# Damo12320/OptixPathtracer

Hardware: AMD Instinct MI355X
Metric: Msamples/sec at 1920x1080, max-depth 8; MSE vs reference (higher is better)
Workload: dtype f32; 1 GPU; BASELINE configs[1]: Diffuse sphere-in-box 1920x1080, 1024 spp, depth 8, 1xMI355X; scene=sphere_box_diffuse, triangles=34570, width=1920, height=1080, max_depth=8, material_mode=lambert, kernel=auto (wavefront), frames_per_launch=128, wavefront_streams=1, parallelism=spp-shard x1, batch_frames=128, queue_bytes=55207544320, queue_budget_bytes=77305217024, bvh_builder=auto (GPU binned SAH + GPU SAH-optimal BVH4 collapse), primary_dedup=True

## Files before the change

optixpathtracer_amd/csrc/pt_device.h:

```cpp
#pragma once
#include "pt_bsdf.h"

namespace pt {

constexpr int kEmptyChild = (int)0x80000000;

struct __align__(16) BNode4 {
    float4 lox, hix, loy, hiy, loz, hiz;
    int4 child;
    int4 pad;
};

__device__ __forceinline__ int leaf_first(int c) { return (~c) >> 3; }
__device__ __forceinline__ int leaf_count(int c) { return ((~c) & 7) + 1; }

struct DevScene {
    const BNode4* nodes;
    const float4* isect;
    const float4* shade;
    const float4* mats;
    const float4* tuv;
    const uint32_t* texels;
    const int4* texinfo;
    int ntri;
// ... 531 lines not shown
                s.h.back = code < 0;
                s.h.orig = ow;
            }
            L->key[lane] = ~0ull;
        }
        __builtin_amdgcn_wave_barrier();
    }
}

template <int ANY, bool STATS, int DEPTH>
__device__ __forceinline__ bool trav_node_step(const DevScene& S, TravState& s, int* __restrict__ stk, int stride,
                                               int* spill, TravStats& ts) {
    if (s.cur >= 0) {
        if (STATS) {
            ts.nodes++;
            ts.lds_nodes += s.cur < S.n_lds;
        }
        float t0, t1, t2, t3;
        int c0, c1, c2, c3;
        const NodeLoad nl = node_load(S, s, s.cur);
#if PT_CYCLE_PROBE
        if (STATS) ts.probe_t = probe_clock(nl.ch.x);
#endif
        node_eval(nl, s, t0, t1, t2, t3, c0, c1, c2, c3);
        if (ANY != kRayAny) {
            cswap(t0, c0, t1, c1);
            cswap(t2, c2, t3, c3);
            cswap(t0, c0, t2, c2);
            cswap(t1, c1, t3, c3);
            cswap(t1, c1, t2, c2);
        }
        if (s.sp > DEPTH - 3) stack_spill<DEPTH, STATS>(s, stk, stride, spill, ts);
        {
            int sp = s.sp;
            stk[sp * stride] = c3;
            sp += c3 != kEmptyChild;
            stk[sp * stride] = c2;
            sp += c2 != kEmptyChild;
            stk[sp * stride] = c1;
            sp += c1 != kEmptyChild;
            s.sp = sp;
        }
        s.cur = c0;
    }
    if (s.cur == kEmptyChild) stack_pop<DEPTH>(s, stk, stride, spill);
    if (s.cur < 0 && s.cur != kEmptyChild && s.leaf == kEmptyChild) {
        s.leaf = s.cur;
        stack_pop<DEPTH>(s, stk, stride, spill);
    }
    return s.cur == kEmptyChild && s.leaf == kEmptyChild;
}

template <int ANY>
__device__ __forceinline__ bool trav_hit_acceptable(const TravState& s, const float4 A, const float4 E1,
                                                    const float4 E2) {
    const float t = is_any<ANY>(s) ? __int_as_float(s.path) : s.h.t;
    return tri_accept(A, E1, E2, s.inv, s.io, t);
}
template <int ANY, bool TEX>
__device__ __forceinline__ bool trav_result_ok(const DevScene& S, const TravState& s) {
    if (s.strict || s.h.tri < 0) return true;
    const int ti = s.h.tri;
    return trav_hit_acceptable<ANY>(s, S.isect[3 * ti], S.isect[3 * ti + 1], S.isect[3 * ti + 2]);
}

template <int ANY>
__device__ __forceinline__ void trav_restart_strict(TravState& s, float tmax_closest) {
    s.cur = 0;
    s.sp = 0;
    s.spc = 0;
    s.leaf = kEmptyChild;
    s.strict = true;
    s.h.tri = -1;
    if (!is_any<ANY>(s)) {
        s.best = tmax_closest;
        s.h.orig = 0x7fffffff;
    }
}

template <int ANY, bool STATS, int DEPTH, bool TEX>
__device__ __forceinline__ bool traverse(const DevScene& S, f3 o, f3 d, float tmin, float tmax, Hit& h,
                                         int* __restrict__ stk, int stride, TravStats& ts) {
    if (STATS) ts.rays++;
    TravState s;
    trav_init(s, o, d, tmin, tmax);
    if (S.ntri > 0) {
        int spill[kSpillDepth];
        while (true) {
            while (!trav_step<ANY, STATS, DEPTH, TEX>(S, s, stk, stride, spill, ts)) {
            }
            if (trav_result_ok<ANY, TEX>(S, s)) break;
            if (STATS) ts.retrace++;
            trav_restart_strict<ANY>(s, tmax);
        }
    }
    h = s.h;
    return s.h.tri >= 0;
}

__device__ __forceinline__ void camera_ray(const DevLaunch& L, int x, int y, f3& o, f3& d) {
    float xs = ((float)x + 0.5f) / (float)L.width;
    float ys = ((float)(y + L.row0) + 0.5f) / (float)L.image_height;
    float ndc[4] = {xs * 2.0f - 1.0f, ys * 2.0f - 1.0f, 1.0f, 1.0f};
    float pv[4], pw[4];
    mat4_mul_vec4(L.inv_proj, ndc, pv);
    float pv0[4] = {pv[0], pv[1], pv[2], 0.0f};
    mat4_mul_vec4(L.inv_view, pv0, pw);
    float d4 = (pw[0] * pw[0] + pw[1] * pw[1]) + (pw[2] * pw[2] + pw[3] * pw[3]);
    float inv = 1.0f / sqrtf(d4);
    d = mk(pw[0] * inv, pw[1] * inv, pw[2] * inv);
    o = mk(L.cam_pos[0], L.cam_pos[1], L.cam_pos[2]);
}

struct SurfaceHit {
    f3 pos, ng;
    Frame fr;
    f3 wo;
    f3 albedo;
    float metallic, roughness;
};

__device__ __forceinline__ void apply_textures(const DevScene& S, int ti, float u, float v, const float4 M1,
                                               const float4 M2, f3& albedo, float& metallic, float& roughness,
                                               f3& Ns) {
    const int at = __float_as_int(M1.z), nt = __float_as_int(M1.w), mt = __float_as_int(M2.x);
    float x, y;
    tri_texcoord(S, ti, u, v, x, y);
    f3 ntex = mk(0.0f, 0.0f, 0.0f);
    if (at >= 0) {
        const float4 c = tex_sample(S, at, x, y, true);
        albedo = albedo * mk(c.x, c.y, c.z);
    }
    if (nt >= 0) {
        const float4 c = tex_sample(S, nt, x, y, false);
        ntex = mk(c.x, c.y, c.z);
    }
    if (mt >= 0) {
        const float4 c = tex_sample(S, mt, x, y, false);
        metallic = c.x;
        roughness = c.y;
    }
    if (ntex.x != 0.0f || ntex.y != 0.0f || ntex.z != 0.0f) {
        f3 d1 = cross(Ns, mk(0.0f, 0.0f, 1.0f));
        f3 d2 = cross(Ns, mk(0.0f, 1.0f, 0.0f));
        f3 T0 = (length(d1) > length(d2)) ? d1 : d2;
        T0 = normalize(T0);
        const f3 B0 = cross(T0, Ns);
        const f3 tn = mk(ntex.x * 2.0f - 1.0f, ntex.y * 2.0f - 1.0f, ntex.z * 2.0f - 1.0f);
        Ns = normalize(mk((T0.x * tn.x + B0.x * tn.y) + Ns.x * tn.z, (T0.y * tn.x + B0.y * tn.y) + Ns.y * tn.z,
                          (T0.z * tn.x + B0.z * tn.y) + Ns.z * tn.z));
    }
}

template <bool TEX>
__device__ __forceinline__ void reconstruct(const DevScene& S, const Hit& h, f3 d, SurfaceHit& s) {
    const int ti = h.tri;
    const float4 A = S.isect[3 * ti];
    const float4 S0 = S.shade[4 * ti], S1 = S.shade[4 * ti + 1], S2 = S.shade[4 * ti + 2], S3 = S.shade[4 * ti + 3];
    const float4 E1 = make_float4(S0.x - A.x, S0.y - A.y, S0.z - A.z, 0.0f);
    const float4 E2 = make_float4(S1.x - A.x, S1.y - A.y, S1.z - A.z, 0.0f);
    const int mi = __float_as_int(S3.w);
    const float4 M0 = S.mats[kMatStride * mi], M1 = S.mats[kMatStride * mi + 1];
    f3 wo_w = normalize(-d);
    f3 v0 = mk(A.x, A.y, A.z), v1 = mk(S0.x, S0.y, S0.z), v2 = mk(S1.x, S1.y, S1.z);
    f3 n0 = mk(S0.w, S1.w, S2.x), n1 = mk(S2.y, S2.z, S2.w), n2 = mk(S3.x, S3.y, S3.z);
    f3 Ng = cross(mk(E1.x, E1.y, E1.z), mk(E2.x, E2.y, E2.z));
    const float u = h.u, v = h.v;
    float w = 1.0f - u - v;
    f3 Ns = mk(w * n0.x + u * n1.x + v * n2.x, w * n0.y + u * n1.y + v * n2.y, w * n0.z + u * n1.z + v * n2.z);
    if (M1.y != kNormalNone) {
        if (TEX && M1.y == kNormalObject) {
            const float4 R0 = S.mats[kMatStride * mi + 3], R1 = S.mats[kMatStride * mi + 4],
                         R2 = S.mats[kMatStride * mi + 5];
            Ns = mk(mat_row_dir(R0, Ns), mat_row_dir(R1, Ns), mat_row_dir(R2, Ns));
        }
        Ns = normalize(Ns);
    }
    if (dot(wo_w, Ng) < 0.0f) Ng = -Ng;
    Ng = normalize(Ng);
    if (dot(Ng, Ns) < 0.0f) Ns = -Ns;
    Ns = normalize(Ns);
    if (h.back) {
        Ns = Ns * -1.0f;
        Ng = Ng * -1.0f;
    }
    s.pos = mk(w * v0.x + u * v1.x + v * v2.x, w * v0.y + u * v1.y + v * v2.y, w * v0.z + u * v1.z + v * v2.z);
    s.ng = Ng;
    s.albedo = mk(M0.x, M0.y, M0.z);
    s.metallic = M0.w;
    s.roughness = M1.x;
    if (TEX) {
        const float4 M2 = S.mats[kMatStride * mi + 2];
        if (M2.y != 0.0f) apply_textures(S, ti, u, v, M1, M2, s.albedo, s.metallic, s.roughness, Ns);
    }
    f3 c1 = cross(Ns, mk(0.0f, 0.0f, 1.0f));
    f3 c2 = cross(Ns, mk(0.0f, 1.0f, 0.0f));
    f3 T = (length(c1) > length(c2)) ? c1 : c2;
    T = normalize(T);
    s.fr.t = T;
    s.fr.b = cross(T, Ns);
    s.fr.n = Ns;
    s.wo = to_local(s.fr, wo_w);
}

struct PathState {
    f3 o, d, beta, radiance;
    uint32_t seed;
    int bounce;
    bool end;
};

__device__ __forceinline__ void path_start(PathState& p, f3 o, f3 d, uint32_t seed) {
    p.o = o;
    p.d = d;
    p.beta = mk(1.0f, 1.0f, 1.0f);
    p.radiance = mk(0.0f, 0.0f, 0.0f);
    p.seed = seed;
    p.bounce = 0;
    p.end = false;
}

__device__ __forceinline__ void debug_record(const DevLaunch& L, int bounce, int prim, const SurfaceHit& sf, f3 beta,
                                             f3 radiance) {
    if (bounce < 1 || bounce > kDebugMaxBounces) return;
    float* r = L.debug + (size_t)(bounce - 1) * kDebugRecordFloats;
    const float v[kDebugRecordFloats] = {__int_as_float(bounce), __int_as_float(prim),
                                         sf.pos.x, sf.pos.y, sf.pos.z, sf.albedo.x, sf.albedo.y, sf.albedo.z,
                                         sf.fr.n.x, sf.fr.n.y, sf.fr.n.z, sf.ng.x, sf.ng.y, sf.ng.z,
                                         sf.roughness, sf.metallic, beta.x, beta.y, beta.z,
                                         radiance.x, radiance.y, radiance.z};
    for (int k = 0; k < kDebugRecordFloats; ++k) r[k] = v[k];
}

__device__ __forceinline__ bool path_alive(const DevLaunch& L, const PathState& p) {
    return !p.end && p.bounce < L.max_bounces && length(p.beta) > 0.00001f;
}

template <int MODE, bool STATS, int DEPTH, bool TEX>
__device__ __forceinline__ void path_segment(const DevScene& S, const DevLaunch& L, PathState& p, int* stk,
                                             int stride, TravStats& ts, bool debug_path) {
    Hit h;
    bool hit = traverse<false, STATS, DEPTH, TEX>(S, p.o, p.d, 0.0f, 100.0f, h, stk, stride, ts);
    if (!hit) {
        p.beta = mk(0, 0, 0);
        p.bounce = 100;
        return;
    }
    p.bounce++;
    if (p.bounce > L.max_bounces) {
        p.end = true;
        return;
    }
    SurfaceHit sf;
    reconstruct<TEX>(S, h, p.d, sf);
    if (debug_path) debug_record(L, p.bounce, __float_as_int(S.isect[3 * h.tri].w), sf, p.beta, p.radiance);
    const bool conductor = rnd(p.seed) < sf.metallic;
    float P = 0.0f;
    int li = 0;
    if (L.n_lights == 1) {
        P = 1.0f;
    } else if (L.n_lights > 1) {
        float r = rnd(p.seed);
        li = (int)(r * (float)L.n_lights);
        if (li >= L.n_lights) li = L.n_lights - 1;
        P = 1.0f / (float)L.n_lights;
    }
    if (P > 0.0f) {
        const DevLight lt = L.lights[li];
        f3 lpos = mk(lt.px, lt.py, lt.pz);
        f3 ldir = lpos - sf.pos;
        f3 ldn = normalize(ldir);
        f3 so = sf.pos + 1e-3f * sf.ng;
        Hit sh;
        bool occluded = traverse<true, STATS, DEPTH, TEX>(S, so, normalize(ldir), 0.0f, length(ldir), sh, stk, stride, ts);
        f3 lds = to_local(sf.fr, ldn);
        if (!occluded) {
            f3 f = bsdf_f<MODE>(p.seed, sf.albedo, sf.roughness, conductor, sf.wo, lds);
            float c = abs_dot(lds, mk(0.0f, 0.0f, 1.0f));
            f3 spectrum = f * c;
            if (!is_zero(spectrum)) {
                f3 dd = sf.pos - lpos;
                float d2 = dd.x * dd.x + dd.y * dd.y + dd.z * dd.z;
                f3 Li = mk(lt.cr, lt.cg, lt.cb) / d2;
                p.radiance = p.radiance + ((p.beta * spectrum) * Li) / (P * 1.0f);
            }
        }
    }
    BSample bs;
    if (p.bounce >= L.max_bounces) {
        p.end = true;
        return;
    }
    if (!bsdf_sample<MODE>(p.seed, sf.albedo, sf.roughness, conductor, sf.wo, bs)) {
        p.end = true;
        return;
    }
    float ac = abs_dot(bs.dir, mk(0.0f, 0.0f, 1.0f));
    p.beta = p.beta * mk(bs.color.x * ac / bs.pdf, bs.color.y * ac / bs.pdf, bs.color.z * ac / bs.pdf);
    f3 off = 1e-3f * sf.ng;
    if (dot(bs.dir, mk(0.0f, 0.0f, 1.0f)) < 0.0f) off = -off;
    p.o = sf.pos + off;
    p.d = normalize(to_world(sf.fr, bs.dir));
}

}
```

optixpathtracer_amd/csrc/pt_wavefront.hip:

```cpp
#include <type_traits>
#include <unordered_map>

#include "pt_internal.h"
#include "pt_lit.h"

namespace pt {

namespace {

constexpr int kBlockWF = 256;
#ifndef PT_TRACE_BLOCK
#define PT_TRACE_BLOCK 256
#endif
constexpr int kBlockTrace = PT_TRACE_BLOCK;
constexpr int kStack = PT_WF_STACK;
#ifndef PT_LDS_NODES
#define PT_LDS_NODES 49
#endif
constexpr int kLdsNodes = PT_LDS_NODES;
#ifndef PT_TRACE_BLOCK_WIDE
#define PT_TRACE_BLOCK_WIDE 768
#endif
#ifndef PT_LDS_NODES_WIDE
#define PT_LDS_NODES_WIDE 150
// ... 16 lines not shown
    if (relay) {
        const unsigned h = __hip_atomic_load(W.cancel_host, __ATOMIC_RELAXED, __HIP_MEMORY_SCOPE_SYSTEM);
        __hip_atomic_fetch_max(W.cancel_seen, h, __ATOMIC_RELAXED, __HIP_MEMORY_SCOPE_AGENT);
    }
    const unsigned v = __hip_atomic_load(W.cancel_seen, __ATOMIC_RELAXED, __HIP_MEMORY_SCOPE_AGENT);
    return __builtin_amdgcn_readfirstlane(v) > W.cancel_epoch;
}
__device__ __forceinline__ bool wf_cancelled(const WFState& W) {
    if (!W.cancel_seen) return false;
    return wf_cancel_poll(W, (blockIdx.x & 63) == 0 && threadIdx.x == 0);
}

__global__ void k_hold(WFState W) {
    if (threadIdx.x != 0 || blockIdx.x != 0) return;
    const unsigned long long t0 = wall_clock64();
    for (int it = 0; it < (1 << 22); ++it) {
        const unsigned h = __hip_atomic_load(W.cancel_host, __ATOMIC_RELAXED, __HIP_MEMORY_SCOPE_SYSTEM);
        if (h > W.cancel_epoch) {
            __hip_atomic_fetch_max(W.cancel_seen, h, __ATOMIC_RELAXED, __HIP_MEMORY_SCOPE_AGENT);
            return;
        }
        if (__hip_atomic_load(W.hold_release, __ATOMIC_RELAXED, __HIP_MEMORY_SCOPE_SYSTEM) != 0u) return;
        if (wall_clock64() - t0 > 1000000000ull) return;
        __builtin_amdgcn_s_sleep(64);
    }
}

__device__ __forceinline__ float4 hit_record(const Hit& h, int path) {
    const float x = __int_as_float(path);
    return h.tri >= 0 ? make_float4(x, h.u, h.v, __int_as_float(h.tri | (h.back ? (int)0x80000000 : 0)))
                      : make_float4(x, 0.0f, 0.0f, __int_as_float(kMissTri));
}

__device__ __forceinline__ unsigned long long wave_sum_u64(unsigned long long v) {
#pragma unroll
    for (int o = 32; o >= 1; o >>= 1) v += __shfl_xor(v, o, 64);
    return v;
}

template <bool STATS>
__device__ __forceinline__ void flush_trav_stats(unsigned long long* counters, const TravStats& ts) {
    if (!STATS || !counters) return;
    const unsigned long long a = wave_sum_u64(ts.nodes), c = wave_sum_u64(ts.tris), d = wave_sum_u64(ts.rays);
    const unsigned long long e = wave_sum_u64(ts.overflow), r = wave_sum_u64(ts.retrace);
    const unsigned long long l = wave_sum_u64(ts.lds_nodes), u = wave_sum_u64(ts.unocc);
    if (lane_id() == 0) {
        atomicAdd(&counters[kCtrNodes], a);
        atomicAdd(&counters[kCtrTriTests], c);
        atomicAdd(&counters[kCtrRays], d);
        atomicAdd(&counters[kCtrStackOverflows], e);
        atomicAdd(&counters[kCtrRetraces], r);
        atomicAdd(&counters[kCtrWaveSteps], (unsigned long long)ts.steps);
        atomicAdd(&counters[kCtrWaveActive], (unsigned long long)ts.active);
        atomicAdd(&counters[kCtrWaveNodeSteps], (unsigned long long)ts.node_steps);
        atomicAdd(&counters[kCtrWaveTriSteps], (unsigned long long)ts.tri_steps);
        atomicAdd(&counters[kCtrWaveRefills], (unsigned long long)ts.refills);
        atomicAdd(&counters[kCtrLdsNodes], l);
        atomicAdd(&counters[kCtrNeeUnoccluded], u);
        for (int k = 0; k < 6; ++k) atomicAdd(&counters[kCtrCoh0 + k], (unsigned long long)ts.coh[k]);
        atomicAdd(&counters[kCtrCohLanes], (unsigned long long)ts.coh_lanes);
    }
}

constexpr int kShadeBuckets = 3;
#ifndef PT_NEE_CLASSES
#define PT_NEE_CLASSES 2
#endif
#ifndef PT_NEE_DARK
#define PT_NEE_DARK 0.5f
#endif
#ifndef PT_NEE_MID
#define PT_NEE_MID 0.7f
#endif
constexpr int kNeeClasses = PT_NEE_CLASSES;
constexpr int kNeeBuckets = 2 + 2 * kNeeClasses;
constexpr int kNeeRegions = kNeeBuckets / 2;
constexpr int kNeeCross = 1;
static_assert(kNeeBuckets <= 8, "a shadow ray's item code holds the NEE bucket in bits 28-30");
constexpr int kCnt = 5 + kNeeBuckets + kShadeBuckets;
constexpr int kCntStride = 32;
enum { kQueue = 0, kShadowQ = 1, kNee0 = 2, kSmp0 = 2 + kNeeBuckets, kPool = 2 + kNeeBuckets + kShadeBuckets, kPoolExt, kPoolSh };
__device__ __forceinline__ int* cnt(const WFState& W, int b, int k) { return W.count + (kCnt * b + k) * kCntStride; }
__device__ __forceinline__ size_t nee_index(const WFState& W, int q, int slot) {
    const size_t r = (size_t)(q >> 1) * W.paths;
    return (q & 1) ? r + W.paths - 1 - slot : r + slot;
}
__device__ __forceinline__ int nee_layered_bucket(int bk, f3 albedo) {
    const float m = fmaxf(fmaxf(albedo.x, albedo.y), albedo.z);
    int cls = 0;
    if (kNeeClasses >= 3 && m < PT_NEE_MID) cls = 1;
    if (kNeeClasses >= 2 && m < PT_NEE_DARK) cls = kNeeClasses - 1;
    return 2 + 2 * cls + (bk - 1);
}
__device__ __forceinline__ size_t smp_index(const WFState& W, int q, int slot) {
    return (size_t)q * W.paths + slot;
}
__device__ __forceinline__ float4* queue_beta(const WFState& W, int b) { return (b & 1) ? W.beta_q : W.beta; }
inline size_t count_bytes(int max_bounces) { return sizeof(int) * kCntStride * kCnt * (size_t)(max_bounces + 2); }

constexpr int kBlockSh = 1024;
constexpr int kWavesSh = kBlockSh / 64;
#ifndef PT_SHA_BLOCK
#define PT_SHA_BLOCK 1024
#endif
constexpr int kBlockShA = PT_SHA_BLOCK, kWavesShA = kBlockShA / 64;
#ifndef PT_SHF_WAVES
#define PT_SHF_WAVES 8
#endif
#ifndef PT_SHF_WAVES_OTHER
#define PT_SHF_WAVES_OTHER 1
#endif
constexpr int shf_waves(int mode) { return (mode == 1 || mode == 3)  ? PT_SHF_WAVES : PT_SHF_WAVES_OTHER; }
#ifndef PT_SHF_BLOCK_DIELECTRIC
#define PT_SHF_BLOCK_DIELECTRIC 256
#endif
#ifndef PT_SHF_BLOCK_CONDUCTOR
#define PT_SHF_BLOCK_CONDUCTOR 256
#endif
#ifndef PT_SHF_BLOCK_LAMBERT
#define PT_SHF_BLOCK_LAMBERT 1024
#endif
constexpr int shf_block(int mode) {
    return mode == 3 ? PT_SHF_BLOCK_DIELECTRIC : mode == 2 ? PT_SHF_BLOCK_CONDUCTOR : PT_SHF_BLOCK_LAMBERT;
}
#ifndef PT_SHB_BLOCK
#define PT_SHB_BLOCK 256
#endif
#ifndef PT_SHB_WAVES
#define PT_SHB_WAVES 4
#endif
#ifndef PT_SMP_WAVES
#define PT_SMP_WAVES 5
#endif
constexpr int kBlockShB = PT_SHB_BLOCK;

template <int WAVES>
__device__ __forceinline__ int block_append(int* counter, bool pred, int* lds) {
    const unsigned long long m = __ballot(pred ? 1 : 0);
    const int prefix = __builtin_amdgcn_mbcnt_hi((uint32_t)(m >> 32), __builtin_amdgcn_mbcnt_lo((uint32_t)m, 0u));
    const int wave = threadIdx.x >> 6;
    if (lane_id() == 0) lds[wave] = __popcll(m);
    __syncthreads();
    if (threadIdx.x == 0) {
        int tot = 0;
        for (int w = 0; w < WAVES; ++w) {
            const int c = lds[w];
            lds[w] = tot;
            tot += c;
        }
        lds[WAVES] = tot > 0 ? atomicAdd(counter, tot) : 0;
    }
    __syncthreads();
    return lds[WAVES] + lds[wave] + prefix;
}

template <int WAVES, int K>
__device__ __forceinline__ int block_append_k(int* counter0, int bucket, int* lds) {
    const int wave = threadIdx.x >> 6;
    unsigned long long mine = 0;
#pragma unroll
    for (int k = 0; k < K; ++k) {
        const unsigned long long m = __ballot(bucket == k ? 1 : 0);
        if (bucket == k) mine = m;
        if (lane_id() == 0) lds[k * WAVES + wave] = __popcll(m);
    }
    __syncthreads();
    if ((int)threadIdx.x < K) {
        const int k = threadIdx.x;
        int tot = 0;
        for (int w = 0; w < WAVES; ++w) {
            const int c = lds[k * WAVES + w];
            lds[k * WAVES + w] = tot;
            tot += c;
        }
        lds[K * WAVES + k] = tot > 0 ? atomicAdd(counter0 + k * kCntStride, tot) : 0;
    }
    __syncthreads();
    if (bucket < 0) return 0;
    const int pre = __builtin_amdgcn_mbcnt_hi((uint32_t)(mine >> 32), __builtin_amdgcn_mbcnt_lo((uint32_t)mine, 0u));
    return lds[K * WAVES + bucket] + lds[bucket * WAVES + wave] + pre;
}

template <int MODE>
__device__ __forceinline__ int shade_bucket(bool conductor, float roughness) {
    if (MODE == kModeDefault && conductor) return 0;
    return sqr(roughness) < 1e-3f ? 1 : 2;
}
constexpr int kItemBits = 28;

__global__ __launch_bounds__(kBlockWF) void k_camera(WFState W, DevLaunch L, uint32_t frame0, int nf, int lean) {
    const int P = L.width * L.height;
    const int Q = P * nf;
    if (wf_cancelled(W)) return;
    if (lean) {
        for (int q = blockIdx.x * blockDim.x + threadIdx.x; q < P; q += gridDim.x * blockDim.x) {
            f3 o, d;
            camera_ray(L, q % L.width, q / L.width, o, d);
            W.ray_o[0][q] = make_float4(o.x, o.y, o.z, __int_as_float(q));
            W.ray_d[0][q] = make_float4(d.x, d.y, d.z, 0.0f);
        }
        if (blockIdx.x == 0 && threadIdx.x == 0) *cnt(W, 0, kQueue) = Q;
        return;
    }
    for (int q = blockIdx.x * blockDim.x + threadIdx.x; q < Q; q += gridDim.x * blockDim.x) {
        const int f = q / P, p = q - f * P;
        const int x = p % L.width, y = p / L.width;
        f3 o, d;
        camera_ray(L, x, y, o, d);
        W.ray_o[0][q] = make_float4(o.x, o.y, o.z, __int_as_float(q));
        W.ray_d[0][q] = make_float4(d.x, d.y, d.z, 0.0f);
        const uint32_t seed = tea16((uint32_t)(L.width * (y + L.row0) + x), frame0 + (uint32_t)f);
        W.beta[q] = make_float4(1.0f, 1.0f, 1.0f, __uint_as_float(seed));
        W.L[q] = make_float4(0.0f, 0.0f, 0.0f, 0.0f);
    }
    if (blockIdx.x == 0 && threadIdx.x == 0) *cnt(W, 0, kQueue) = Q;
}

#ifndef PT_REFILL_MIN
#define PT_REFILL_MIN 16
#endif
constexpr int kRefillMin = PT_REFILL_MIN;

#ifndef PT_TRI_BATCH
#define PT_TRI_BATCH 20
#endif

__device__ __forceinline__ void wave_slice(int n, int& first, int& end) {
    const int wave = (int)((blockIdx.x * blockDim.x + threadIdx.x) >> 6);
    const int nwaves = (int)((gridDim.x * blockDim.x) >> 6);
    const int per = (n + nwaves - 1) / nwaves;
    first = min(n, wave * per);
    end = min(n, first + per);
}

typedef float pt_v4f __attribute__((ext_vector_type(4)));
__device__ __forceinline__ float4 ldqs(const float4* p) {
    const pt_v4f v = __builtin_nontemporal_load(reinterpret_cast<const pt_v4f*>(p));
    return make_float4(v.x, v.y, v.z, v.w);
}
__device__ __forceinline__ void stqs(float4* p, float4 v) {
    __builtin_nontemporal_store(pt_v4f{v.x, v.y, v.z, v.w}, reinterpret_cast<pt_v4f*>(p));
}

#ifndef PT_TRACE_POOL
#define PT_TRACE_POOL 60
#endif
#ifndef PT_TRACE_POOL_X
#define PT_TRACE_POOL_X 60
#endif
#ifndef PT_POOL_CHUNK
#define PT_POOL_CHUNK 512
#endif
#ifndef PT_POOL_MIN_PER_WAVE
#define PT_POOL_MIN_PER_WAVE 2048
#endif
__device__ __forceinline__ bool pool_pays(int n) {
    const long long nwaves = (long long)((gridDim.x * blockDim.x) >> 6);
    return (long long)n >= nwaves * PT_POOL_MIN_PER_WAVE;
}
struct RayPool {
    int* ctr = nullptr;
    int begin = 0, end = 0;
};

struct NoCommit {
    template <class T>
    __device__ void operator()(const T&) const {}
};
template <int ANY, bool STATS, bool TEX, int BLK, class Fetch, class Finish, class Commit = NoCommit>
__device__ __forceinline__ void trace_range(const DevScene& S, int next, int end, int* stk, TriBatchLds* tri_lds,
                                            TravStats& ts, const WFState& W, Fetch fetch, Finish finish,
                                            Commit commit = Commit{}, RayPool pool = RayPool{}) {
    using Tok = decltype(finish(0, *static_cast<const TravState*>(nullptr)));
    constexpr bool kSplit = !std::is_void_v<Tok>;
    using TokS = std::conditional_t<kSplit, Tok, int>;
    int spill[kSpillDepth];
    TravState st;
    int ri = -1;
    bool done = false;
    next = __builtin_amdgcn_readfirstlane(next);
    end = __builtin_amdgcn_readfirstlane(end);
    uint32_t npoll = 0;
    int* pctr = pool.ctr;
    if (W.cancel_seen && wf_cancel_poll(W, false)) {
        end = next;
        pctr = nullptr;
    }
    while (true) {
        if ((int)__popcll(__ballot(ri < 0 || done)) >= kRefillMin || next >= end) {
            if (W.cancel_seen && (++npoll & 15) == 0 &&
                wf_cancel_poll(W, (npoll & 63) == 0 && (blockIdx.x & 7) == 0 && threadIdx.x == 0)) {
                end = next;
                pctr = nullptr;
            }
            if (pctr && next >= end) {
                int base = 0;
                if ((threadIdx.x & 63) == 0) base = atomicAdd(pctr, PT_POOL_CHUNK);
                base = __builtin_amdgcn_readfirstlane(__shfl(base, 0, 64));
                next = min(pool.begin + base, pool.end);
                end = min(next + PT_POOL_CHUNK, pool.end);
                if (next >= pool.end) pctr = nullptr;
            }
#if PT_CYCLE_PROBE
            const uint64_t c0 = probe_clock();
#else
            if (STATS) ts.refills++;
// ... 16 lines not shown
                if (STATS) ts.rays++;
                done = S.ntri <= 0;
            }
            next = min(next + (int)__popcll(m), end);
            if constexpr (kSplit) {
                if (fin) commit(tok);
            }
#if PT_CYCLE_PROBE
            if (STATS) ts.refills += (uint32_t)(probe_clock(st.best) - c0);
#endif
        }
        const bool active = ri >= 0 && !done;
        const unsigned long long act = __ballot(active);
        if (!act && !__ballot(ri >= 0)) break;
        const int n_act = __popcll(act);
        const int n_leaf = __popcll(__ballot(active && st.leaf != kEmptyChild));
        const int n_node = __popcll(__ballot(active && st.cur >= 0));
        const bool tri_ok = n_leaf >= min(PT_TRI_BATCH, n_act) || 2 * n_node < n_act;
        if (STATS) {
            ts.steps++;
#if !PT_CYCLE_PROBE
            ts.active += n_act;
            ts.node_steps += n_node > 0;
            ts.tri_steps += tri_ok && n_leaf > 0;
#endif
        }
#if PT_CYCLE_PROBE
        const uint64_t c1 = probe_clock();
#endif
        if (tri_ok && n_leaf > 0) {
            wave_tri_batch<ANY, STATS, TEX>(S, st, active && st.leaf != kEmptyChild, tri_lds, ts);
            if (active && is_any<ANY>(st) && st.h.tri >= 0) done = true;
        }
#if PT_CYCLE_PROBE
        const uint64_t c2 = probe_clock(st.best);
        if (STATS) ts.tri_steps += (uint32_t)(c2 - c1);
#endif
        if (STATS) {
            const bool g = active && !done && st.cur >= S.n_lds;
            unsigned long long rem = __ballot(g);
            if (rem) {
                ts.coh_lanes += (uint32_t)__popcll(rem);
                int distinct = 0;
                while (rem) {
                    const int node = __shfl(st.cur, __ffsll((long long)rem) - 1, 64);
                    rem &= ~__ballot(g && st.cur == node);
                    ++distinct;
                }
                ts.coh[distinct <= 2 ? distinct - 1 : distinct <= 4 ? 2 : distinct <= 8 ? 3 : distinct <= 16 ? 4 : 5]++;
            }
        }
        if (active && !done && trav_node_step<ANY, STATS, kStack>(S, st, stk, BLK, spill, ts)) done = true;
#if PT_CYCLE_PROBE
        if (STATS) {
            const uint64_t c4 = probe_clock(st.cur);
            const unsigned long long ml = __ballot(ts.probe_t > c2);
            const uint64_t tl = ml ? (uint64_t)__shfl((long long)ts.probe_t, __ffsll((long long)ml) - 1, 64) : c2;
            ts.active += (uint32_t)(tl - c2);
            ts.node_steps += (uint32_t)(c4 - tl);
        }
#endif
    }
}

template <int ANY, bool STATS, bool TEX, int BLK, class Fetch, class Finish, class Commit = NoCommit>
__device__ __forceinline__ void trace_queue(DevScene S, int first, int end, TravStats& ts, const WFState& W, Fetch fetch,
                                            Finish finish, Commit commit = Commit{}, RayPool pool = RayPool{}) {
    constexpr int kNodes = lds_nodes_of<BLK>();
    __shared__ int stack[kStack * BLK];
    __shared__ BNode4 top[kNodes > 0 ? kNodes : 1];
    __shared__ TriBatchLds tri_batch[BLK / 64];
    stage_top_nodes<kNodes>(S, top);
    trace_range<ANY, STATS, TEX, BLK>(S, first, end, stack + threadIdx.x, tri_batch + (threadIdx.x >> 6), ts, W, fetch,
                                      finish, commit, pool);
}

template <int ANY, bool STATS, bool TEX, int BLK, class Fetch, class Finish>
__device__ __forceinline__ void trace_slice(const DevScene& S, int n, TravStats& ts, const WFState& W, Fetch fetch,
                                            Finish finish, int* pool_ctr) {
    int next, end;
    RayPool pool;
    pool.end = n;
    if (PT_TRACE_POOL_X > 0 && pool_pays(n)) {
        pool.ctr = pool_ctr;
        pool.begin = n - (int)((long long)n * PT_TRACE_POOL_X / 100);
    } else {
        pool.begin = n;
    }
    wave_slice(pool.begin, next, end);
    trace_queue<ANY, STATS, TEX, BLK>(S, next, end, ts, W, fetch, finish, NoCommit{}, pool);
}

template <bool STATS, bool TEX, int BLK = kBlockTrace>
__global__ __launch_bounds__(BLK, wf_waves(TEX)) void k_extend(DevScene S, WFState W, int b, int dup,
                                                                  int copies, unsigned long long* counters) {
    const int n = *cnt(W, b, kQueue);
    const int n_trace = n / dup;
    const float4* ro = W.ray_o[b & 1];
    const float4* rd = W.ray_d[b & 1];
    TravStats ts;
    trace_slice<kRayClosest, STATS, TEX, BLK>(
        S, n_trace, ts, W,
        [&](int ri, TravState& st) {
            const float4 a = ro[ri], c = rd[ri];
            trav_init(st, mk(a.x, a.y, a.z), mk(c.x, c.y, c.z), 0.0f, 100.0f);
            st.path = __float_as_int(a.w);
        },
        [&](int ri, const TravState& st) {
            for (int k = 0; k < copies; ++k) {
                float4* rec = W.hit + ri + (size_t)k * n_trace;
                *rec = hit_record(st.h, st.path + k * n_trace);
            }
        }, cnt(W, b, kPoolExt));
    if (blockIdx.x == 0 && threadIdx.x == 0 && counters) {
        atomicAdd(&counters[kCtrSegments], (unsigned long long)n);
        atomicAdd(&counters[kCtrTraceRays], (unsigned long long)n_trace);
        atomicAdd(&counters[kCtrTraceBytes], (32ull + 16ull * (unsigned long long)copies) * (unsigned long long)n_trace);
    }
    flush_trav_stats<STATS>(counters, ts);
}

__device__ __forceinline__ Hit decode_hit(float4 hv) {
    Hit h;
    const int code = __float_as_int(hv.w);
    h.t = hv.x;
    h.u = hv.y;
    h.v = hv.z;
    h.back = code != kMissTri && (code & (int)0x80000000);
    h.tri = code == kMissTri ? -1 : (code & 0x7fffffff);
    return h;
}

__device__ __forceinline__ float pick_light(const DevLaunch& L, uint32_t& seed, int& li) {
    li = 0;
    if (L.n_lights == 1) return 1.0f;
    if (L.n_lights <= 0) return 0.0f;
    float r = rnd(seed);
    li = (int)(r * (float)L.n_lights);
    if (li >= L.n_lights) li = L.n_lights - 1;
    return 1.0f / (float)L.n_lights;
}

__device__ __forceinline__ bool continue_path(const SurfaceHit& sf, const BSample& bs, f3& beta, f3& o, f3& d,
                                              int next_bounce, int max_bounces) {
    float ac = abs_dot(bs.dir, mk(0.0f, 0.0f, 1.0f));
    beta = beta * mk(bs.color.x * ac / bs.pdf, bs.color.y * ac / bs.pdf, bs.color.z * ac / bs.pdf);
    f3 off = 1e-3f * sf.ng;
    if (dot(bs.dir, mk(0.0f, 0.0f, 1.0f)) < 0.0f) off = -off;
    o = sf.pos + off;
    d = normalize(to_world(sf.fr, bs.dir));
    return next_bounce < max_bounces && length(beta) > 0.00001f;
}

__device__ __forceinline__ int lit_cell(const DevLaunch& L, const Hit& h) {
    const uint32_t w = L.lit_tri[h.tri];
    const int k = lit_level(w);
    return k == kLitNoCells ? -1 : (int)(lit_first(w) + lit_cell_index(k, h.u, h.v));
}
__device__ __forceinline__ bool lit_bit(const DevLaunch& L, int li, int cell) {
    return (L.lit_bits[(size_t)li * L.lit_words + ((uint32_t)cell >> 5)] >> (cell & 31)) & 1u;
}
__device__ __forceinline__ void lit_count_wave(bool answered, int* lds) {
    const unsigned long long m = __ballot(answered ? 1 : 0);
    if (lane_id() == 0) lds[threadIdx.x >> 6] = __popcll(m);
}
template <int WAVES, int SLOT = kCtrLitAnswers>
__device__ __forceinline__ void lit_count_block(const DevLaunch& L, const int* lds) {
    if (threadIdx.x != 0 || !L.counters) return;
    int tot = 0;
    for (int w = 0; w < WAVES; ++w) tot += lds[w];
    if (tot > 0) atomicAdd(&L.counters[SLOT], (unsigned long long)tot);
}
template <bool TEX>
__device__ __forceinline__ bool occ_answers(const DevScene& S, int t, f3 o, f3 d, float tmax) {
    if (t < 0) return false;
    const float4 A = S.isect[3 * t], E1 = S.isect[3 * t + 1], E2 = S.isect[3 * t + 2];
    float th, uh, vh;
    bool bk;
    if (!tri_test(A, E1, E2, o, d, 0.0f, tmax, th, uh, vh, bk)) return false;
    if (TEX && __float_as_int(E2.w) != 0) return false;
    const f3 inv = safe_inv(d);
    return tri_accept(A, E1, E2, inv, mk(o.x * inv.x, o.y * inv.y, o.z * inv.z), th);
}

__device__ __forceinline__ int vis0_index(const DevLaunch& L, int path, int li) {
    const int P1 = L.width * L.height;
    return li * P1 + path % P1;
}

template <bool TEX>
__global__ __launch_bounds__(kBlockWF) void k_shadow0_setup(DevScene S, DevLaunch L, WFState W) {
    const int P1 = L.width * L.height;
    const int nl = L.n_lights;
    const int n = P1 * nl;
    if (wf_cancelled(W)) return;
    for (int k = blockIdx.x * blockDim.x + threadIdx.x; k < n; k += gridDim.x * blockDim.x) {
        const int li = k / P1, p = k - li * P1;
        const Hit h = decode_hit(W.hit[p]);
        float4 so = make_float4(0.0f, 0.0f, 0.0f, __int_as_float(k)), sd = make_float4(0.0f, 0.0f, 1.0f, 0.0f);
        if (h.tri >= 0) {
            const float4 c = W.ray_d[0][p];
            SurfaceHit sf;
            reconstruct<TEX>(S, h, mk(c.x, c.y, c.z), sf);
            const DevLight lt = L.lights[li];
            const f3 ldir = mk(lt.px, lt.py, lt.pz) - sf.pos;
            const f3 o = sf.pos + 1e-3f * sf.ng;
            const f3 d = normalize(ldir);
            so = make_float4(o.x, o.y, o.z, __int_as_float(k));
            sd = make_float4(d.x, d.y, d.z, length(ldir));
        }
        W.sh_o[k] = so;
        W.sh_d[k] = sd;
    }
    if (blockIdx.x == 0 && threadIdx.x == 0) *cnt(W, 0, kShadowQ) = n;
}

template <int MODE, bool TEX, bool SHADE0>
__global__ __launch_bounds__(shf_block(MODE), shf_waves(MODE)) void k_shade_fused(DevScene S, DevLaunch L, WFState W, int b, int vis0) {
    constexpr bool shade0 = SHADE0;
    constexpr bool kBetaQ = MODE == kModeLambert;
    constexpr bool kShareOrigin = MODE == kModeLambert;
    constexpr int kBlock = shf_block(MODE), kWaves = kBlock / 64;
    const int n = *cnt(W, b, kQueue);
    const float4* rd = W.ray_d[b & 1];
    float4* no = W.ray_o[(b + 1) & 1];
    float4* nd = W.ray_d[(b + 1) & 1];
    __shared__ int lds_sh[kWaves + 1], lds_q[kWaves + 1];
    __shared__ int lds_lit[kWaves];
    constexpr bool kOcc = MODE == kModeLambert;
    __shared__ int lds_occ[kOcc ? kWaves : 1];
    const bool lit = !vis0 && L.lit_tri;
    const bool occ = kOcc && lit && L.occ_tab;
    if (blockIdx.x == 0 && threadIdx.x == 0 && L.counters) atomicAdd(&L.counters[kCtrShadeItems], (unsigned long long)n);
    if ((int)(blockIdx.x * kBlock) >= n) return;
    {
        const int i = (int)(blockIdx.x * kBlock + threadIdx.x);
        const bool valid = i < n && !wf_cancelled(W);
        bool emit_shadow = false, emit_next = false, lit_answer = false;
        f3 so, sdir, contrib, o, d, beta;
        uint32_t seed = 0;
        float stmax = 0.0f;
        int path = 0;
        int occ_t = -1;
        const int P1 = L.width * L.height;
        float4 l0 = make_float4(0.0f, 0.0f, 0.0f, 0.0f);
        if (valid) {
            const float4 hv = ldqs(W.hit + i);
            const float4 c_q = shade0 ? make_float4(0.0f, 0.0f, 0.0f, 0.0f) : ldqs(rd + i);
            const float4 bv_q = (!shade0 && kBetaQ) ? ldqs(queue_beta(W, b) + i) : make_float4(0.0f, 0.0f, 0.0f, 0.0f);
            path = __float_as_int(hv.x);
            const Hit h = decode_hit(hv);
            if (h.tri >= 0) {
                const int lit_c = lit ? lit_cell(L, h) : -1;
                const float4 c = shade0 ? ldqs(rd + path % P1) : c_q;
                d = mk(c.x, c.y, c.z);
                SurfaceHit sf;
                reconstruct<TEX>(S, h, d, sf);
                if (shade0) {
                    seed = tea16((uint32_t)(path % P1 + L.width * L.row0), L.frame_base + (uint32_t)(path / P1));
                    beta = mk(1.0f, 1.0f, 1.0f);
                } else {
                    float4 bv = kBetaQ ? bv_q : ldqs(W.beta + path);
                    seed = __float_as_uint(bv.w);
                    beta = mk(bv.x, bv.y, bv.z);
                }
                if (path == debug_path_id(L)) {
                    const float4 l = shade0 ? l0 : W.L[path];
                    debug_record(L, b + 1, __float_as_int(S.isect[3 * h.tri].w), sf, beta, mk(l.x, l.y, l.z));
                }
                const bool conductor = rnd(seed) < sf.metallic;
                int li;
                const float P = pick_light(L, seed, li);
                if (P > 0.0f) {
                    const DevLight lt = L.lights[li];
                    f3 lpos = mk(lt.px, lt.py, lt.pz);
                    f3 ldir = lpos - sf.pos;
                    f3 ldn = normalize(ldir);
                    f3 lds = to_local(sf.fr, ldn);
                    f3 f = bsdf_f<MODE>(seed, sf.albedo, sf.roughness, conductor, sf.wo, lds);
                    f3 spectrum = f * abs_dot(lds, mk(0.0f, 0.0f, 1.0f));
                    if (!is_zero(spectrum)) {
                        f3 dd = sf.pos - lpos;
                        float d2 = dd.x * dd.x + dd.y * dd.y + dd.z * dd.z;
                        f3 Li = mk(lt.cr, lt.cg, lt.cb) / d2;
                        contrib = ((beta * spectrum) * Li) / (P * 1.0f);
                        lit_answer = lit_c >= 0 && dot(ldir, sf.ng) > kLitDelta && lit_bit(L, li, lit_c);
                        if (vis0 || lit_answer) {
                            if (lit_answer || W.vis[vis0_index(L, path, li)]) {
                                const float4 l = shade0 ? l0 : W.L[path];
                                l0 = make_float4(l.x + contrib.x, l.y + contrib.y, l.z + contrib.z, 0.0f);
                                if (!shade0) W.L[path] = l0;
                            }
                        } else {
                            so = sf.pos + 1e-3f * sf.ng;
                            sdir = normalize(ldir);
                            stmax = length(ldir);
                            emit_shadow = true;
                            if (kOcc && occ && lit_c >= 0 && dot(ldir, sf.ng) > kLitDelta)
                                occ_t = L.occ_tab[li * (int)L.lit_cells + lit_c];
                        }
                    }
                }
                BSample bs;
                if (b + 1 < L.max_bounces &&
                    bsdf_sample<MODE>(seed, sf.albedo, sf.roughness, conductor, sf.wo, bs)) {
                    emit_next = continue_path(sf, bs, beta, o, d, b + 1, L.max_bounces);
                    if (!kBetaQ) stqs(W.beta + path, make_float4(beta.x, beta.y, beta.z, __uint_as_float(seed)));
                }
            }
        }
        if (shade0 && valid) W.L[path] = l0;
        if (lit) lit_count_wave(lit_answer, lds_lit);
        const int qi = block_append<kWaves>(cnt(W, b + 1, kQueue), emit_next, lds_q);
        if (lit) lit_count_block<kWaves>(L, lds_lit);
        if (emit_next) {
            stqs(no + qi, make_float4(o.x, o.y, o.z, __int_as_float(path)));
            stqs(nd + qi, make_float4(d.x, d.y, d.z, 0.0f));
            if (kBetaQ) stqs(queue_beta(W, b + 1) + qi, make_float4(beta.x, beta.y, beta.z, __uint_as_float(seed)));
        }
        if constexpr (kOcc) {
            if (occ) {
                bool answered = false;
                if (occ_t >= 0) answered = occ_answers<TEX>(S, occ_t, (kShareOrigin && emit_next) ? o : so, sdir, stmax);
                if (answered) emit_shadow = false;
                lit_count_wave(answered, lds_occ);
            }
        }
        const int si = block_append<kWaves>(cnt(W, b, kShadowQ), emit_shadow, lds_sh);
        if constexpr (kOcc) {
            if (occ) lit_count_block<kWaves, kCtrOccAnswers>(L, lds_occ);
        }
        if (emit_shadow) {
            const bool share = kShareOrigin && emit_next;
            if (!share) stqs(W.sh_o + si, make_float4(so.x, so.y, so.z, __int_as_float(path)));
            stqs(W.sh_d + si, make_float4(sdir.x, sdir.y, sdir.z, stmax));
            stqs(W.sh_c + si, make_float4(contrib.x, contrib.y, contrib.z, __int_as_float(share ? qi : -1)));
        }
    }
}

template <int MODE, bool TEX>
__global__ __launch_bounds__(shf_block(MODE), 1) void k_shade0_pixel(DevScene S, DevLaunch L, WFState W, int nf) {
    constexpr bool kBetaQ = MODE == kModeLambert;
    constexpr int kBlock = shf_block(MODE), kWaves = kBlock / 64;
    const int P1 = L.width * L.height;
    __shared__ int lds_q[kWaves + 1];
    if (blockIdx.x == 0 && threadIdx.x == 0 && L.counters)
        atomicAdd(&L.counters[kCtrShadeItems], (unsigned long long)P1 * (unsigned long long)nf);
    if ((int)(blockIdx.x * kBlock) >= P1) return;
    const int p = (int)(blockIdx.x * kBlock + threadIdx.x);
    const bool valid = p < P1 && !wf_cancelled(W);
    int tri = -1;
    SurfaceHit sf;
    if (valid) {
        const float4 hv = W.hit[p];
        const Hit h = decode_hit(hv);
        tri = h.tri;
        if (tri >= 0) {
            const float4 c = W.ray_d[0][p];
            reconstruct<TEX>(S, h, mk(c.x, c.y, c.z), sf);
        }
    }
    const int dbg = debug_path_id(L);
    float4* no = W.ray_o[1];
    float4* nd = W.ray_d[1];
    for (int f = 0; f < nf; ++f) {
        const int path = f * P1 + p;
        bool emit_next = false;
        f3 o, d, beta = mk(1.0f, 1.0f, 1.0f);
        uint32_t seed = 0;
        float4 l0 = make_float4(0.0f, 0.0f, 0.0f, 0.0f);
        if (valid && tri >= 0) {
            seed = tea16((uint32_t)(p + L.width * L.row0), L.frame_base + (uint32_t)f);
            if (path == dbg) debug_record(L, 1, __float_as_int(S.isect[3 * tri].w), sf, beta, mk(0.0f, 0.0f, 0.0f));
            const bool conductor = rnd(seed) < sf.metallic;
            int li;
            const float P = pick_light(L, seed, li);
            if (P > 0.0f) {
                const DevLight lt = L.lights[li];
                f3 lpos = mk(lt.px, lt.py, lt.pz);
                f3 lds = to_local(sf.fr, normalize(lpos - sf.pos));
                f3 fv = bsdf_f<MODE>(seed, sf.albedo, sf.roughness, conductor, sf.wo, lds);
                f3 spectrum = fv * abs_dot(lds, mk(0.0f, 0.0f, 1.0f));
                if (!is_zero(spectrum) && W.vis[vis0_index(L, path, li)]) {
                    f3 dd = sf.pos - lpos;
                    float d2 = dd.x * dd.x + dd.y * dd.y + dd.z * dd.z;
                    f3 Li = mk(lt.cr, lt.cg, lt.cb) / d2;
                    f3 contrib = ((beta * spectrum) * Li) / (P * 1.0f);
                    l0 = make_float4(0.0f + contrib.x, 0.0f + contrib.y, 0.0f + contrib.z, 0.0f);
                }
            }
            BSample bs;
            if (1 < L.max_bounces && bsdf_sample<MODE>(seed, sf.albedo, sf.roughness, conductor, sf.wo, bs)) {
                emit_next = continue_path(sf, bs, beta, o, d, 1, L.max_bounces);
                if (!kBetaQ) stqs(W.beta + path, make_float4(beta.x, beta.y, beta.z, __uint_as_float(seed)));
            }
        }
        if (valid) stqs(W.L + path, l0);
        const int qi = block_append<kWaves>(cnt(W, 1, kQueue), emit_next, lds_q);
        if (emit_next) {
            stqs(no + qi, make_float4(o.x, o.y, o.z, __int_as_float(path)));
            stqs(nd + qi, make_float4(d.x, d.y, d.z, 0.0f));
            if (kBetaQ) stqs(queue_beta(W, 1) + qi, make_float4(beta.x, beta.y, beta.z, __uint_as_float(seed)));
        }
    }
}

template <bool STATS, bool TEX, int BLK = kBlockTrace>
__global__ __launch_bounds__(BLK, wf_waves(TEX)) void k_trace_pair(DevScene S, WFState W, int b,
                                                                      unsigned long long* counters) {
    const int n_ext = *cnt(W, b + 1, kQueue);
    const int n_sh = *cnt(W, b, kShadowQ);
    const float4* ro = W.ray_o[(b + 1) & 1];
    const float4* rd = W.ray_d[(b + 1) & 1];
    TravStats ts;
    auto fetch = [&](int i, TravState& st) {
        if (i < n_ext) {
            const float4 a = ldqs(ro + i), c = ldqs(rd + i);
            trav_init(st, mk(a.x, a.y, a.z), mk(c.x, c.y, c.z), 0.0f, 100.0f);
            st.path = __float_as_int(a.w);
        } else {
            const int j = i - n_ext;
            const float4 c = ldqs(W.sh_d + j), k = ldqs(W.sh_c + j);
            const int q = __float_as_int(k.w);
            const float4 a = ldqs(q >= 0 ? ro + q : W.sh_o + j);
            trav_init(st, mk(a.x, a.y, a.z), mk(c.x, c.y, c.z), 0.0f, c.w);
            st.any = true;
            st.h.orig = __float_as_int(a.w);
            st.h.t = k.x;
            st.h.u = k.y;
            st.h.v = k.z;
        }
    };
    struct NeeAdd {
        float4* p;
        float4 v;
        float x, y, z;
    };
    auto finish = [&](int i, const TravState& st) -> NeeAdd {
        NeeAdd a{nullptr, make_float4(0.0f, 0.0f, 0.0f, 0.0f), 0.0f, 0.0f, 0.0f};
        const Hit& h = st.h;
        if (i < n_ext) stqs(W.hit + i, hit_record(h, st.path));
        __builtin_amdgcn_sched_barrier(0);
        if (STATS && i >= n_ext && h.tri < 0) ts.unocc++;
        if (i >= n_ext && h.tri < 0) {
            a.p = W.L + h.orig;
            a.v = *a.p;
            a.x = h.t;
            a.y = h.u;
            a.z = h.v;
        }
        return a;
    };
    auto commit = [&](const NeeAdd& a) {
        if (a.p) *a.p = make_float4(a.v.x + a.x, a.v.y + a.y, a.v.z + a.z, 0.0f);
    };
    int first, end;
    const int n_all = n_ext + n_sh;
    RayPool pool;
    if (PT_TRACE_POOL > 0 && pool_pays(n_all)) {
        pool.ctr = cnt(W, b, kPool);
        pool.end = n_all;
        pool.begin = n_all - (int)((long long)n_all * PT_TRACE_POOL / 100);
    } else {
        pool.begin = pool.end = n_all;
    }
    wave_slice(pool.begin, first, end);
    trace_queue<kRayMixed, STATS, TEX, BLK>(S, first, end, ts, W, fetch, finish, commit, pool);
    if (blockIdx.x == 0 && threadIdx.x == 0 && counters) {
        atomicAdd(&counters[kCtrSegments], (unsigned long long)n_ext);
        atomicAdd(&counters[kCtrShadowRays], (unsigned long long)n_sh);
        atomicAdd(&counters[kCtrTraceRays], (unsigned long long)(n_ext + n_sh));
        atomicAdd(&counters[kCtrTraceBytes], 48ull * (unsigned long long)(n_ext + n_sh));
        atomicAdd(&counters[kCtrPairRays], (unsigned long long)(n_ext + n_sh));
        atomicAdd(&counters[kCtrPairBytes], 48ull * (unsigned long long)(n_ext + n_sh));
        atomicAdd(&counters[kCtrPairShadowRays], (unsigned long long)n_sh);
    }
    flush_trav_stats<STATS>(counters, ts);
}

template <int MODE, bool TEX>
__global__ __launch_bounds__(kBlockShA) void k_shade_a(DevScene S, DevLaunch L, WFState W, int b, int vis0) {
    const int n = *cnt(W, b, kQueue);
    const float4* rd = W.ray_d[b & 1];
    __shared__ int lds_sh[kWavesShA + 1];
    __shared__ int lds_nee[kNeeBuckets * (kWavesShA + 1)], lds_smp[kShadeBuckets * (kWavesShA + 1)];
    __shared__ int lds_lit[kWavesShA], lds_occ[kWavesShA];
    const bool lit = !vis0 && L.lit_tri;
    const bool occ = lit && L.occ_tab;
    if ((int)(blockIdx.x * kBlockShA) >= n) return;
// ... 564 lines not shown
```

Baseline: 1776 Msamples/sec.

## Merge shade queue appends into one two-queue block scan and hoist loads early

Combines the next-ray and shadow-ray block appends into one scan, so a block runs two __syncthreads barriers instead of four and the two atomics are issued by different waves at once. In Lambert non-texture mode, the triangle records, light record and occlusion-candidate triangle are loaded before they are needed, so their latency overlaps other work. The occlusion test moves before the append, and the radiance accumulation is deferred to the end of the kernel. In exchange, more values are live at once, which raises register pressure, and the origin handling around kShareOrigin becomes more involved.

```diff
diff --git a/optixpathtracer_amd/csrc/pt_device.h b/optixpathtracer_amd/csrc/pt_device.h
--- a/optixpathtracer_amd/csrc/pt_device.h
+++ b/optixpathtracer_amd/csrc/pt_device.h
@@ -707,11 +707,24 @@
     }
 }
 
+struct TriRecords {
+    float4 A, S0, S1, S2, S3;
+};
+__device__ __forceinline__ TriRecords tri_records(const DevScene& S, int ti) {
+    TriRecords r;
+    r.A = S.isect[3 * ti];
+    r.S0 = S.shade[4 * ti];
+    r.S1 = S.shade[4 * ti + 1];
+    r.S2 = S.shade[4 * ti + 2];
+    r.S3 = S.shade[4 * ti + 3];
+    return r;
+}
+
 template <bool TEX>
-__device__ __forceinline__ void reconstruct(const DevScene& S, const Hit& h, f3 d, SurfaceHit& s) {
+__device__ __forceinline__ void reconstruct(const DevScene& S, const Hit& h, f3 d, const TriRecords& r, SurfaceHit& s) {
     const int ti = h.tri;
-    const float4 A = S.isect[3 * ti];
-    const float4 S0 = S.shade[4 * ti], S1 = S.shade[4 * ti + 1], S2 = S.shade[4 * ti + 2], S3 = S.shade[4 * ti + 3];
+    const float4 A = r.A;
+    const float4 S0 = r.S0, S1 = r.S1, S2 = r.S2, S3 = r.S3;
     const float4 E1 = make_float4(S0.x - A.x, S0.y - A.y, S0.z - A.z, 0.0f);
     const float4 E2 = make_float4(S1.x - A.x, S1.y - A.y, S1.z - A.z, 0.0f);
     const int mi = __float_as_int(S3.w);
@@ -756,6 +769,10 @@
     s.fr.b = cross(T, Ns);
     s.fr.n = Ns;
     s.wo = to_local(s.fr, wo_w);
+}
+template <bool TEX>
+__device__ __forceinline__ void reconstruct(const DevScene& S, const Hit& h, f3 d, SurfaceHit& s) {
+    reconstruct<TEX>(S, h, d, tri_records(S, h.tri), s);
 }
 
 struct PathState {
diff --git a/optixpathtracer_amd/csrc/pt_wavefront.hip b/optixpathtracer_amd/csrc/pt_wavefront.hip
--- a/optixpathtracer_amd/csrc/pt_wavefront.hip
+++ b/optixpathtracer_amd/csrc/pt_wavefront.hip
@@ -192,6 +192,36 @@
     }
     __syncthreads();
     return lds[WAVES] + lds[wave] + prefix;
+}
+
+template <int WAVES>
+__device__ __forceinline__ void block_append2(int* counter_a, bool pred_a, int* counter_b, bool pred_b, int* lds,
+                                              int* slot_a, int* slot_b) {
+    static_assert(WAVES >= 2, "queue b is summed by the second wave's first thread");
+    const unsigned long long ma = __ballot(pred_a ? 1 : 0), mb = __ballot(pred_b ? 1 : 0);
+    const int prefix_a = __builtin_amdgcn_mbcnt_hi((uint32_t)(ma >> 32), __builtin_amdgcn_mbcnt_lo((uint32_t)ma, 0u));
+    const int prefix_b = __builtin_amdgcn_mbcnt_hi((uint32_t)(mb >> 32), __builtin_amdgcn_mbcnt_lo((uint32_t)mb, 0u));
+    const int wave = threadIdx.x >> 6;
+    int* la = lds;
+    int* lb = lds + WAVES + 1;
+    if (lane_id() == 0) {
+        la[wave] = __popcll(ma);
+        lb[wave] = __popcll(mb);
+    }
+    __syncthreads();
+    if (lane_id() == 0 && wave < 2) {
+        int* l = wave ? lb : la;
+        int tot = 0;
+        for (int w = 0; w < WAVES; ++w) {
+            const int c = l[w];
+            l[w] = tot;
+            tot += c;
+        }
+        l[WAVES] = tot > 0 ? atomicAdd(wave ? counter_b : counter_a, tot) : 0;
+    }
+    __syncthreads();
+    *slot_a = la[WAVES] + la[wave] + prefix_a;
+    *slot_b = lb[WAVES] + lb[wave] + prefix_b;
 }
 
 template <int WAVES, int K>
@@ -514,11 +544,11 @@
     return next_bounce < max_bounces && length(beta) > 0.00001f;
 }
 
-__device__ __forceinline__ int lit_cell(const DevLaunch& L, const Hit& h) {
-    const uint32_t w = L.lit_tri[h.tri];
+__device__ __forceinline__ int lit_cell(uint32_t w, const Hit& h) {
     const int k = lit_level(w);
     return k == kLitNoCells ? -1 : (int)(lit_first(w) + lit_cell_index(k, h.u, h.v));
 }
+__device__ __forceinline__ int lit_cell(const DevLaunch& L, const Hit& h) { return lit_cell(L.lit_tri[h.tri], h); }
 __device__ __forceinline__ bool lit_bit(const DevLaunch& L, int li, int cell) {
     return (L.lit_bits[(size_t)li * L.lit_words + ((uint32_t)cell >> 5)] >> (cell & 31)) & 1u;
 }
@@ -534,15 +564,18 @@
     if (tot > 0) atomicAdd(&L.counters[SLOT], (unsigned long long)tot);
 }
 template <bool TEX>
-__device__ __forceinline__ bool occ_answers(const DevScene& S, int t, f3 o, f3 d, float tmax) {
-    if (t < 0) return false;
-    const float4 A = S.isect[3 * t], E1 = S.isect[3 * t + 1], E2 = S.isect[3 * t + 2];
+__device__ __forceinline__ bool occ_answers(float4 A, float4 E1, float4 E2, f3 o, f3 d, float tmax) {
     float th, uh, vh;
     bool bk;
     if (!tri_test(A, E1, E2, o, d, 0.0f, tmax, th, uh, vh, bk)) return false;
     if (TEX && __float_as_int(E2.w) != 0) return false;
     const f3 inv = safe_inv(d);
     return tri_accept(A, E1, E2, inv, mk(o.x * inv.x, o.y * inv.y, o.z * inv.z), th);
+}
+template <bool TEX>
+__device__ __forceinline__ bool occ_answers(const DevScene& S, int t, f3 o, f3 d, float tmax) {
+    if (t < 0) return false;
+    return occ_answers<TEX>(S.isect[3 * t], S.isect[3 * t + 1], S.isect[3 * t + 2], o, d, tmax);
 }
 
 __device__ __forceinline__ int vis0_index(const DevLaunch& L, int path, int li) {
@@ -587,10 +620,11 @@
     const float4* rd = W.ray_d[b & 1];
     float4* no = W.ray_o[(b + 1) & 1];
     float4* nd = W.ray_d[(b + 1) & 1];
-    __shared__ int lds_sh[kWaves + 1], lds_q[kWaves + 1];
+    __shared__ int lds_app[2 * (kWaves + 1)];
     __shared__ int lds_lit[kWaves];
     constexpr bool kOcc = MODE == kModeLambert;
     __shared__ int lds_occ[kOcc ? kWaves : 1];
+    constexpr bool kEarly = MODE == kModeLambert && !TEX;
     const bool lit = !vis0 && L.lit_tri;
     const bool occ = kOcc && lit && L.occ_tab;
     if (blockIdx.x == 0 && threadIdx.x == 0 && L.counters) atomicAdd(&L.counters[kCtrShadeItems], (unsigned long long)n);
@@ -598,7 +632,10 @@
     {
         const int i = (int)(blockIdx.x * kBlock + threadIdx.x);
         const bool valid = i < n && !wf_cancelled(W);
-        bool emit_shadow = false, emit_next = false, lit_answer = false;
+        bool emit_shadow = false, emit_next = false, lit_answer = false, answered = false;
+        bool add = false;
+        constexpr bool kLateAdd = MODE == kModeLambert && !shade0;
+        float4 lrad = make_float4(0.0f, 0.0f, 0.0f, 0.0f);
         f3 so, sdir, contrib, o, d, beta;
         uint32_t seed = 0;
         float stmax = 0.0f;
@@ -612,12 +649,20 @@
             const float4 bv_q = (!shade0 && kBetaQ) ? ldqs(queue_beta(W, b) + i) : make_float4(0.0f, 0.0f, 0.0f, 0.0f);
             path = __float_as_int(hv.x);
             const Hit h = decode_hit(hv);
+            if (!shade0) d = mk(c_q.x, c_q.y, c_q.z);
+            if (!shade0 && kBetaQ) {
+                seed = __float_as_uint(bv_q.w);
+                beta = mk(bv_q.x, bv_q.y, bv_q.z);
+            }
             if (h.tri >= 0) {
-                const int lit_c = lit ? lit_cell(L, h) : -1;
+                const uint32_t lit_t = lit ? L.lit_tri[h.tri] : 0u;
+                TriRecords tr;
+                if (kEarly) tr = tri_records(S, h.tri);
+                const int lit_c = lit ? lit_cell(lit_t, h) : -1;
                 const float4 c = shade0 ? ldqs(rd + path % P1) : c_q;
                 d = mk(c.x, c.y, c.z);
                 SurfaceHit sf;
-                reconstruct<TEX>(S, h, d, sf);
+                if (!kEarly) reconstruct<TEX>(S, h, d, sf);
                 if (shade0) {
                     seed = tea16((uint32_t)(path % P1 + L.width * L.row0), L.frame_base + (uint32_t)(path / P1));
                     beta = mk(1.0f, 1.0f, 1.0f);
@@ -626,15 +671,19 @@
                     seed = __float_as_uint(bv.w);
                     beta = mk(bv.x, bv.y, bv.z);
                 }
+                const float coin = rnd(seed);
+                int li;
+                const float P = pick_light(L, seed, li);
+                DevLight lt;
+                if (kEarly && P > 0.0f) lt = L.lights[li];
+                if (kEarly) reconstruct<TEX>(S, h, d, tr, sf);
                 if (path == debug_path_id(L)) {
                     const float4 l = shade0 ? l0 : W.L[path];
                     debug_record(L, b + 1, __float_as_int(S.isect[3 * h.tri].w), sf, beta, mk(l.x, l.y, l.z));
                 }
-                const bool conductor = rnd(seed) < sf.metallic;
-                int li;
-                const float P = pick_light(L, seed, li);
+                const bool conductor = coin < sf.metallic;
                 if (P > 0.0f) {
-                    const DevLight lt = L.lights[li];
+                    if (!kEarly) lt = L.lights[li];
                     f3 lpos = mk(lt.px, lt.py, lt.pz);
                     f3 ldir = lpos - sf.pos;
                     f3 ldn = normalize(ldir);
@@ -646,22 +695,30 @@
                         float d2 = dd.x * dd.x + dd.y * dd.y + dd.z * dd.z;
                         f3 Li = mk(lt.cr, lt.cg, lt.cb) / d2;
                         contrib = ((beta * spectrum) * Li) / (P * 1.0f);
-                        lit_answer = lit_c >= 0 && dot(ldir, sf.ng) > kLitDelta && lit_bit(L, li, lit_c);
+                        const bool side = lit_c >= 0 && dot(ldir, sf.ng) > kLitDelta;
+                        lit_answer = side && lit_bit(L, li, lit_c);
                         if (vis0 || lit_answer) {
-                            if (lit_answer || W.vis[vis0_index(L, path, li)]) {
+                            add = lit_answer || W.vis[vis0_index(L, path, li)];
+                            if (add && !kLateAdd) {
                                 const float4 l = shade0 ? l0 : W.L[path];
                                 l0 = make_float4(l.x + contrib.x, l.y + contrib.y, l.z + contrib.z, 0.0f);
                                 if (!shade0) W.L[path] = l0;
                             }
                         } else {
-                            so = sf.pos + 1e-3f * sf.ng;
+                            if (!kShareOrigin) so = sf.pos + 1e-3f * sf.ng;
                             sdir = normalize(ldir);
                             stmax = length(ldir);
                             emit_shadow = true;
-                            if (kOcc && occ && lit_c >= 0 && dot(ldir, sf.ng) > kLitDelta)
-                                occ_t = L.occ_tab[li * (int)L.lit_cells + lit_c];
+                            if (kOcc && occ && side) occ_t = L.occ_tab[li * (int)L.lit_cells + lit_c];
                         }
                     }
+                }
+                float4 cA, cE1, cE2;
+                if constexpr (kOcc) {
+                    const int ct = occ_t >= 0 ? occ_t : 0;
+                    cA = S.isect[3 * ct];
+                    cE1 = S.isect[3 * ct + 1];
+                    cE2 = S.isect[3 * ct + 2];
                 }
                 BSample bs;
                 if (b + 1 < L.max_bounces &&
@@ -669,35 +726,38 @@
                     emit_next = continue_path(sf, bs, beta, o, d, b + 1, L.max_bounces);
                     if (!kBetaQ) stqs(W.beta + path, make_float4(beta.x, beta.y, beta.z, __uint_as_float(seed)));
                 }
+                if (kShareOrigin && emit_shadow && !emit_next) o = sf.pos + 1e-3f * sf.ng;
+                if constexpr (kOcc) {
+                    if (occ_t >= 0) answered = occ_answers<TEX>(cA, cE1, cE2, kShareOrigin ? o : so, sdir, stmax);
+                    if (answered) emit_shadow = false;
+                }
+                if (kLateAdd && add) lrad = W.L[path];
             }
         }
         if (shade0 && valid) W.L[path] = l0;
         if (lit) lit_count_wave(lit_answer, lds_lit);
-        const int qi = block_append<kWaves>(cnt(W, b + 1, kQueue), emit_next, lds_q);
+        if constexpr (kOcc) {
+            if (occ) lit_count_wave(answered, lds_occ);
+        }
+        int qi, si;
+        block_append2<kWaves>(cnt(W, b + 1, kQueue), emit_next, cnt(W, b, kShadowQ), emit_shadow, lds_app, &qi, &si);
         if (lit) lit_count_block<kWaves>(L, lds_lit);
+        if constexpr (kOcc) {
+            if (occ) lit_count_block<kWaves, kCtrOccAnswers>(L, lds_occ);
+        }
         if (emit_next) {
             stqs(no + qi, make_float4(o.x, o.y, o.z, __int_as_float(path)));
             stqs(nd + qi, make_float4(d.x, d.y, d.z, 0.0f));
             if (kBetaQ) stqs(queue_beta(W, b + 1) + qi, make_float4(beta.x, beta.y, beta.z, __uint_as_float(seed)));
         }
-        if constexpr (kOcc) {
-            if (occ) {
-                bool answered = false;
-                if (occ_t >= 0) answered = occ_answers<TEX>(S, occ_t, (kShareOrigin && emit_next) ? o : so, sdir, stmax);
-                if (answered) emit_shadow = false;
-                lit_count_wave(answered, lds_occ);
-            }
-        }
-        const int si = block_append<kWaves>(cnt(W, b, kShadowQ), emit_shadow, lds_sh);
-        if constexpr (kOcc) {
-            if (occ) lit_count_block<kWaves, kCtrOccAnswers>(L, lds_occ);
-        }
         if (emit_shadow) {
             const bool share = kShareOrigin && emit_next;
-            if (!share) stqs(W.sh_o + si, make_float4(so.x, so.y, so.z, __int_as_float(path)));
+            const f3 org = kShareOrigin ? o : so;
+            if (!share) stqs(W.sh_o + si, make_float4(org.x, org.y, org.z, __int_as_float(path)));
             stqs(W.sh_d + si, make_float4(sdir.x, sdir.y, sdir.z, stmax));
             stqs(W.sh_c + si, make_float4(contrib.x, contrib.y, contrib.z, __int_as_float(share ? qi : -1)));
         }
+        if (kLateAdd && add) W.L[path] = make_float4(lrad.x + contrib.x, lrad.y + contrib.y, lrad.z + contrib.z, 0.0f);
     }
 }
 
```

New measurement: 1788 Msamples/sec, median of 6. About the same (+0.7%).
